# bxh1/VIDO-SLAM

Hardware: AMD Instinct MI355X
Metric: frames/sec end-to-end (flow+depth+track+local-BA) at 640x480; BA iters/sec (higher is better)
Workload: dtype f32

## Files before the change

include/vido_c.h:

```cpp
#ifndef VIDO_C_H
#define VIDO_C_H
#include <stdint.h>
#include <stddef.h>
#ifdef __cplusplus
extern "C" {
#endif

#define VIDO_OK              0
#define VIDO_E_INVALID      -1
#define VIDO_E_NO_DEVICE    -2
#define VIDO_E_HIP          -3
#define VIDO_E_CAPACITY     -4
#define VIDO_E_NOMEM        -5

#define VIDO_MAX_LEVELS 16

typedef struct vido_ctx vido_ctx;

typedef struct vido_keypoint { float x, y, size, angle, response; int32_t octave; } vido_keypoint;

typedef struct vido_config {
    int32_t device;
    int32_t width, height;
    int32_t max_batch;
// ... 152 lines not shown
int vido_conv1x1_set_arith(int arith);
int vido_conv1x1_range_flag(vido_ctx* ctx, int reset);
int vido_conv1x1_bias_act(vido_ctx* ctx, const float* x, const float* w_packed, const float* bias, const float* residual, float* y, int cin, int cout, int hw, float slope);
int vido_deconv2x2_supported(int n, int cin, int cout, int h, int w);
int vido_deconv2x2_bias_act(vido_ctx* ctx, const float* x, const float* w_packed, const float* bias, float* y, int n, int cin, int cout, int h, int w, float slope);
int vido_conv1x1_bias_up2_act(vido_ctx* ctx, const float* x, const float* w_packed, const float* bias, const float* residual_half, float* y, int cin, int cout, int h, int w, float slope);

int vido_conv_kxk_c2(vido_ctx* ctx, const float* x, const float* w, const float* bias, const float* residual, float* y, int cin, int k, int h, int w_);
int vido_conv1x1_skinny(vido_ctx* ctx, const float* x, const float* w_packed, const float* bias, const float* residual, float* y, int cin, int cout, long long hw, float slope);

int vido_conv_direct_supported(int cin, int cout, int h, int w, int kh, int kw, int sh, int sw, int ph, int pw);
long long vido_conv_direct_packed_floats(int cin, int cout, int kh, int kw);
int vido_conv_direct_pack(const float* w, int cin, int cout, int kh, int kw, float* w_packed);
int vido_conv_direct_bias_act(vido_ctx* ctx, const float* x, const float* w_packed, const float* bias, float* y, int n, int cin, int cout, int h, int w,
                              int kh, int kw, int sh, int sw, int ph, int pw, float slope);

int vido_wino3x3_supported(int cin, int cout, int h, int w);
int vido_wino3x3_fills_chip(int n, int cout, int h, int w, int min_wgs);
long long vido_wino3x3_packed_floats(int cin, int cout);
int vido_wino3x3_pack(const float* w, int cin, int cout, float* u_packed);
int vido_wino3x3_bias_act(vido_ctx* ctx, const float* x, const float* u_packed, const float* bias, float* y, int n, int cin, int cout, int h, int w, float slope);
int vido_wino3x3_form(int n, int cin, int cout, int h, int w);
int vido_fc_h_splitk(int rows, int k, int outs);
int vido_fc_h(vido_ctx* ctx, const float* x, const void* w_packed, const float* bias, float* part, float* y, int rows, int k, int outs, float slope);
int vido_conv3x3_h_supported(int n, int cin, int cout, int h, int w);
int vido_conv3x3_h_workgroups(int n, int cout, int h, int w);
int vido_conv3x3_h_bias_act(vido_ctx* ctx, const float* x, const void* w_packed, const float* bias, float* y, int n, int cin, int cout, int h, int w, float slope);
long long vido_wino3x3_packed_floats_form(int cin, int cout, int form);
int vido_wino3x3_pack_form(const float* w, int cin, int cout, int form, float* u_packed);
int vido_wino3x3_bias_act_form(vido_ctx* ctx, const float* x, const float* u_packed, const float* bias, float* y, int n, int cin, int cout, int h, int w, float slope, int form);
int vido_gconv3x3_supported(int H, int W, int cpg_in, int cpg_out);
int64_t vido_gconv3x3_packed_size(int groups, int cpg_in, int cpg_out);
int vido_gconv3x3_bias_act(vido_ctx* ctx, const float* x, const float* in_bias, const float* w_packed, const float* bias, float* y, int groups, int cpg_in, int cpg_out, int H, int W, float slope);
int vido_gconv3x3_s2_supported(int H, int W, int cpg_in, int cpg_out);
int vido_gconv3x3_s2_bias_act(vido_ctx* ctx, const float* x, const float* w_packed, const float* bias, float* y, int groups, int cpg_in, int cpg_out, int H, int W, float slope);
int vido_lfn_reg_front(vido_ctx* ctx, const float* im1, const float* im2, const float* flow, const float* mean, float scale, int B, int C, int H, int W, float* out, int out_channels);
int vido_lfn_reg_tail(vido_ctx* ctx, const float* dist, const float* flow, const float* wx, const float* bx, const float* wy, const float* by, int B, int K, int H, int W, float* out);
int vido_roi_align(vido_ctx* ctx, const float* feat, int B, int C, int H, int W, const float* rois, int n_rois,
                   float spatial_scale, int pooled_h, int pooled_w, int sampling_ratio, float* out, int on_device);
int vido_nms(vido_ctx* ctx, const float* boxes_xyxy, const float* scores, int n, float thresh, int32_t* keep_out,
             int32_t* n_keep, int on_device);
int vido_nms_grouped(vido_ctx* ctx, const float* boxes_xyxy, const float* scores, const int32_t* groups, int n, float thresh,
                     int32_t* keep_out, int32_t* n_keep, int on_device);
int vido_nms_segments(vido_ctx* ctx, const float* boxes_xyxy, const int32_t* groups, const int32_t* seg_off, const int32_t* seg_n, int n_seg, int max_n, int total,
                      float thresh, int32_t* keep_out, int32_t* n_keep);
int vido_roi_align_fpn(vido_ctx* ctx, const float* const feat[4], const int H[4], const int W[4], const float scale[4], int C, const float* boxes, const int32_t* level,
                       int n, int pooled_h, int pooled_w, int sampling_ratio, float* out);
int vido_nchw_to_nhwc(vido_ctx* ctx, const float* src, int B, int C, int H, int W, float* dst);
int vido_roi_align_fpn_nhwc(vido_ctx* ctx, const float* const feat[4], const int H[4], const int W[4], const float scale[4], int C, const float* boxes, const int32_t* level,
                            int n, int pooled_h, int pooled_w, int sampling_ratio, float* out);
int vido_bawin_create(vido_ctx* ctx, int cap_frames, int cap_features);
int vido_bawin_push_frame(vido_ctx* ctx, int frame, int n, const double* meas, const float* xyz, const int32_t* asso);
int vido_bawin_set_labels(vido_ctx* ctx, int n, const int32_t* quads);
int vido_bawin_solve(vido_ctx* ctx, int start, int N, vido_ba_problem* prob, vido_ba_result* res, int32_t* n_obs_out, int32_t* n_pt_out);
int vido_bawin_read_points(vido_ctx* ctx, int frame, int n, float* xyz_out);
int vido_rpn_select(vido_ctx* ctx, int n_levels, const float* const* logits, const float* const* deltas, const int* h, const int* w, const int* stride, const float* cell_anchors,
                    int A, int K, int img_w, int img_h, float* boxes_out, float* scores_out, int32_t* n_out);
int vido_rpn_merge(vido_ctx* ctx, const float* boxes, const float* scores, const int32_t* keep, const int32_t* cnt, int n_levels, int K, int post_nms_top_n, int n_final,
                   float* out_boxes, float* out_scores, int32_t* n_valid);
int vido_det_class_sort(vido_ctx* ctx, const float* prob, const float* deltas, const float* proposals, const float* objectness, int N, int nc, float thresh, const float weights[4],
                        int img_w, int img_h, float* seg_boxes, int32_t* order, int32_t* seg_n);
int vido_det_select(vido_ctx* ctx, const float* prob, const float* seg_boxes, const int32_t* order, const int32_t* keep, const int32_t* cnt, int N, int nc, int detections_per_img, int cap,
                    int32_t* scratch, float* out_boxes, float* out_scores, int64_t* out_labels, int32_t* n_det);
int vido_mask_label_image(vido_ctx* ctx, const float* masks, const float* boxes, const int64_t* labels, int n, int M, int padding, float thresh, int H, int W, uint8_t* out);
int vido_box_decode(vido_ctx* ctx, const float* deltas, const float* boxes, int n, int k, const float weights[4],
                    float* out, int on_device);
// ... 62 lines not shown
```

vido-slam_amd/csrc/conv3x3h.hip:

```cpp
#include "common.hpp"
#include <type_traits>

namespace {
typedef float f32x16 __attribute__((ext_vector_type(16)));
typedef float f32x2 __attribute__((ext_vector_type(2)));
typedef _Float16 f16x8 __attribute__((ext_vector_type(8)));
typedef _Float16 f16x2 __attribute__((ext_vector_type(2)));
typedef unsigned u32x4 __attribute__((ext_vector_type(4)));

#define C3_OOB 0x40000000u
#define C3_WSLOT 24576
#define C3_RBW 3
#define C3_WPIX(BR) (((BR) + 2) * 18)
#define C3_XP(BR) ((16 * C3_WPIX(BR) + 511) / 512)
#define C3_RAW(BR) (C3_XP(BR) * 8 * 256)
#define C3_PLANE(BR) (C3_WPIX(BR) * 32)
#define C3_PBUF(BR) (2 * C3_PLANE(BR))
#define C3_LDS(BR) (C3_RBW * C3_WSLOT + C3_RAW(BR) + 2 * C3_PBUF(BR))

struct C3Args { const float* x; const void* wp; const float* bias; float* y; int N, Cin, Cout, H, W, nby, nbx, mt, total, nchunk; float slope; unsigned xbytes, wbytes; unsigned* range_flag; };

template <int RPW, int CG>
__global__ __launch_bounds__(512) void k_conv3x3_h(C3Args A)
{
    constexpr int BR = 16 / CG, MT = 32 * RPW * CG, WPIX = C3_WPIX(BR), XP = C3_XP(BR), RAWB = C3_RAW(BR), PLANE = C3_PLANE(BR), PBUF = C3_PBUF(BR), CK = (WPIX * 8 + 511) / 512, NMM = 9 * RPW, NRD = 2 * RPW + 2;
    extern __shared__ __attribute__((aligned(16))) char c3_lds[];
    char* L = c3_lds;
    const int tid = threadIdx.x, lane = tid & 63, w = __builtin_amdgcn_readfirstlane(tid >> 6);
    const int per = gridDim.x >> 3, item = (blockIdx.x & 7) * per + (blockIdx.x >> 3);
    if (item >= A.total) return;
    const int nt = item / A.mt, mtile = item - nt * A.mt, m0 = mtile * MT;
    const int bpi = A.nby * A.nbx, n = nt / bpi, brem = nt - n * bpi, by = brem / A.nbx, bx = brem - by * A.nbx, Y0 = by * BR, X0 = bx * 16;
    const int rp = CG == 1 ? w : (w & 3), rb0 = CG == 1 ? 0 : RPW * (w >> 2);
    const int hw = A.H * A.W, nsteps = A.nchunk * 3;

    const __amdgpu_buffer_rsrc_t wr = __builtin_amdgcn_make_buffer_rsrc((void*)A.wp, 0, A.wbytes, 0x00020000);
    const unsigned avo = 16u * (unsigned)lane;
    unsigned abase[3], avq[3];
#pragma unroll
    for (int q = 0; q < 3; q++) { const int i = w + 8 * q, rb = i / 6, rem = i - 6 * rb; abase[q] = 1024u * (unsigned)(((m0 >> 5) + rb) * A.nchunk * 18 + rem); avq[q] = rb < RPW * CG ? avo : 0x80000000u; }
    unsigned xvo[11];
#pragma unroll
    for (int j = 0; j < XP; j++) {
        const int e = 64 * (8 * j + w) + lane, ch = e / WPIX, rem = e - ch * WPIX, row = rem / 18, col = rem - row * 18, gy = Y0 - 1 + row, gx = X0 - 1 + col;
        xvo[j] = (e < 16 * WPIX && gy >= 0 && gy < A.H && gx >= 0 && gx < A.W) ? 4u * (unsigned)(ch * hw + gy * A.W + gx) : C3_OOB;
    }
    const unsigned ximg = 4u * (unsigned)n * (unsigned)A.Cin * (unsigned)hw, xchunk = 64u * (unsigned)hw;
    char* const RAW = L + C3_RBW * C3_WSLOT;
    char* const PL = RAW + RAWB;
    auto issue_w = [&](int s, int slot) {
        char* S = L + slot * C3_WSLOT + w * 1024;
        const unsigned so = 6144u * (unsigned)s;
#pragma unroll
        for (int q = 0; q < 3; q++) __builtin_amdgcn_raw_ptr_buffer_load_lds(wr, (__attribute__((address_space(3))) void*)(S + q * 8192), 16, avq[q], abase[q] + so, 0, 0);
    };
    auto issue_x = [&](int c) {
        const unsigned so = ximg + xchunk * (unsigned)c;
        const __amdgpu_buffer_rsrc_t xc = __builtin_amdgcn_make_buffer_rsrc((void*)((const char*)A.x + so), 0, A.xbytes - so, 0x00020000);
#pragma unroll
        for (int j = 0; j < XP; j++) __builtin_amdgcn_raw_ptr_buffer_load_lds(xc, (__attribute__((address_space(3))) void*)(RAW + (8 * j + w) * 256), 4, xvo[j], 0, 0, 0);
    };
    float xmax = 0.f;
    const f32x2 k2048 = {2048.f, 2048.f};
    auto convert = [&](int buf) {
        const float* R = (const float*)RAW;
        unsigned* P = (unsigned*)(PL + buf * PBUF);
#pragma unroll
        for (int k = 0; k < CK; k++) {
            const int idx = tid + 512 * k;
            if (k < CK - 1 || idx < WPIX * 8) {
                const int q = idx / WPIX, pix = idx - q * WPIX;
                const f32x2 v = {R[(2 * q) * WPIX + pix], R[(2 * q + 1) * WPIX + pix]};
                const f16x2 h = __builtin_convertvector(v, f16x2);
                f32x2 vs, r;
                asm("v_pk_mul_f32 %0, %1, %2" : "=v"(vs) : "v"(v), "v"(k2048));
                asm("v_fma_mix_f32 %0, %1, %2, %3 op_sel_hi:[1,0,0]" : "=v"(r.x) : "v"(h), "s"(-2048.f), "v"(vs.x));
                asm("v_fma_mix_f32 %0, %1, %2, %3 op_sel:[1,0,0] op_sel_hi:[1,0,0]" : "=v"(r.y) : "v"(h), "s"(-2048.f), "v"(vs.y));
                const f16x2 l = __builtin_convertvector(r, f16x2);
                P[pix * 8 + q] = __builtin_bit_cast(unsigned, h); P[PLANE / 4 + pix * 8 + q] = __builtin_bit_cast(unsigned, l);
                xmax = __builtin_fmaxf(__builtin_fmaxf(xmax, __builtin_fabsf(v.x)), __builtin_fabsf(v.y));
            }
        }
    };

    f32x16 acc[RPW], acl[RPW];
#pragma unroll
    for (int rb = 0; rb < RPW; rb++)
#pragma unroll
        for (int r = 0; r < 16; r++) { acc[rb][r] = 0.f; acl[rb][r] = 0.f; }
    typedef const __attribute__((address_space(3))) char* lds_c;
    const unsigned a_lane = 16u * (unsigned)lane;
    const unsigned b_lane = (unsigned)(C3_RBW * C3_WSLOT + RAWB) + 32u * (unsigned)((2 * rp + ((lane & 31) >> 4)) * 18 + (lane & 15)) + 16u * (unsigned)(lane >> 5);

    issue_x(0); issue_w(0, 0); issue_w(min(1, nsteps - 1), 1);
    asm volatile("s_waitcnt vmcnt(6) lgkmcnt(0)\n\ts_barrier" ::: "memory");
    convert(0);
    int slot = 0;
    u32x4 a[2][RPW][2], b[2][2];
    auto step = [&](auto dy_c, auto nbuf_c, int pbuf, auto&& copies) {
        constexpr int dy = decltype(dy_c)::value, NBUF = decltype(nbuf_c)::value;
        lds_c Ab = (lds_c)(L + slot * C3_WSLOT) + a_lane;
        lds_c Bb = (lds_c)L + b_lane + pbuf * PBUF + dy * (18 * 32);
        auto ld = [&](int dx, int set) {
#pragma unroll
            for (int rb = 0; rb < RPW; rb++)
#pragma unroll
                for (int pl = 0; pl < 2; pl++) a[set][rb][pl] = *(const __attribute__((address_space(3))) u32x4*)(Ab + (((rb0 + rb) * 3 + dx) * 2 + pl) * 1024);
#pragma unroll
            for (int pl = 0; pl < 2; pl++) b[set][pl] = *(const __attribute__((address_space(3))) u32x4*)(Bb + dx * 32 + pl * PLANE);
        };
        __builtin_amdgcn_sched_barrier(0);
        ld(0, 0);
        copies();
#pragma unroll
        for (int dx = 0; dx < 3; dx++) {
            if (dx < 2) ld(dx + 1, (dx + 1) & 1);
#pragma unroll
            for (int term = 0; term < 3; term++) {
                constexpr int PA[3] = {0, 1, 0}, PB[3] = {1, 0, 0};
#pragma unroll
                for (int rb = 0; rb < RPW; rb++) {
                    f32x16& d = term == 2 ? acc[rb] : acl[rb];
                    d = __builtin_amdgcn_mfma_f32_32x32x16_f16(__builtin_bit_cast(f16x8, a[dx & 1][rb][PA[term]]), __builtin_bit_cast(f16x8, b[dx & 1][PB[term]]), d, 0, 0, 0);
                }
            }
        }
        __builtin_amdgcn_sched_group_barrier(0x100, NRD, 0);
#pragma unroll
        for (int i = 0; i < NMM; i++) {
            __builtin_amdgcn_sched_group_barrier(0x008, 1, 0);
            if (i < 2 * NRD) __builtin_amdgcn_sched_group_barrier(0x100, 1, 0);
            if (i >= 1 && i < 1 + NBUF) __builtin_amdgcn_sched_group_barrier(0x020, 1, 0);
        }
        __builtin_amdgcn_sched_barrier(0);
    };
    for (int c = 0; c < A.nchunk; c++) {
        const int pbuf = c & 1, cn = min(c + 1, A.nchunk - 1);
        asm volatile("s_waitcnt vmcnt(3) lgkmcnt(0)\n\ts_barrier" ::: "memory");
        step(std::integral_constant<int, 0>{}, std::integral_constant<int, 3 + XP>{}, pbuf, [&] { const int sf = slot == 0 ? C3_RBW - 1 : slot - 1; issue_w(min(3 * c + 2, nsteps - 1), sf); issue_x(cn); });
        slot = slot + 1 == C3_RBW ? 0 : slot + 1;
        asm volatile("s_waitcnt vmcnt(%0) lgkmcnt(0)\n\ts_barrier" :: "n"(3 + XP) : "memory");
        step(std::integral_constant<int, 1>{}, std::integral_constant<int, 3>{}, pbuf, [&] { const int sf = slot == 0 ? C3_RBW - 1 : slot - 1; issue_w(min(3 * c + 3, nsteps - 1), sf); });
        slot = slot + 1 == C3_RBW ? 0 : slot + 1;
        asm volatile("s_waitcnt vmcnt(3) lgkmcnt(0)\n\ts_barrier" ::: "memory");
        step(std::integral_constant<int, 2>{}, std::integral_constant<int, 3>{}, pbuf, [&] { const int sf = slot == 0 ? C3_RBW - 1 : slot - 1; issue_w(min(3 * c + 4, nsteps - 1), sf); });
        convert(pbuf ^ 1);
        slot = slot + 1 == C3_RBW ? 0 : slot + 1;
    }
    asm volatile("s_waitcnt vmcnt(0) lgkmcnt(0)" ::: "memory");
#pragma unroll
    for (int rb = 0; rb < RPW; rb++) acc[rb] += acl[rb] * 0x1p-11f;
    if (!(xmax < 65504.f) && A.range_flag) atomicOr(A.range_flag, 1u);

    const float* wsc = (const float*)((const char*)A.wp + (size_t)A.nchunk * 16 * 18 * A.Cout * 2);
    const int p = lane & 31, Y = Y0 + 2 * rp + (p >> 4), X = X0 + (p & 15);
    const bool inside = Y < A.H && X < A.W;
    float* yb = A.y + (size_t)n * A.Cout * hw + (size_t)Y * A.W + X;
#pragma unroll
    for (int rb = 0; rb < RPW; rb++) {
        float bv[16], sv[16];
#pragma unroll
        for (int r = 0; r < 16; r++) { const int co = m0 + 32 * (rb0 + rb) + 8 * (r >> 2) + 4 * (lane >> 5) + (r & 3); bv[r] = A.bias ? A.bias[co] : 0.f; sv[r] = wsc[co]; }
        if (inside) {
#pragma unroll
            for (int r = 0; r < 16; r++) {
                const int co = m0 + 32 * (rb0 + rb) + 8 * (r >> 2) + 4 * (lane >> 5) + (r & 3);
                const float v = acc[rb][r] * sv[r] + bv[r];
                yb[(size_t)co * hw] = fmaxf(v, v * A.slope);
            }
        }
    }
}
}

extern "C" {

int vido_conv3x3_h_supported(int n, int cin, int cout, int h, int w)
{
    const long long cp = (cin + 15) / 16 * 16;
    return n >= 1 && cin >= 1 && (cout == 32 || cout == 64 || (cout >= 128 && cout % 128 == 0)) && h >= 1 && w >= 1 && 4ll * n * cin * h * w < (1ll << 30) && 4ll * n * cout * h * w < (1ll << 30)
           && 36ll * cp * cout < (1ll << 31);
}

#define C3_MIN16 190
static int c3_block_rows(int n, int cout, int h, int w)
{
    static const int force = [] { const char* e = getenv("VIDO_CONV3X3_H_ROWS"); return e ? atoi(e) : 0; }();
    if (cout == 32) return 16;
    if (force == 16 || force == 8) return force;
    const int mt = cout >= 128 ? cout / 128 : 1;
    return n * ((h + 15) / 16) * ((w + 15) / 16) * mt >= C3_MIN16 ? 16 : 8;
}
int vido_conv3x3_h_workgroups(int n, int cout, int h, int w) { const int br = c3_block_rows(n, cout, h, w); return n * ((h + br - 1) / br) * ((w + 15) / 16) * (cout >= 128 ? cout / 128 : 1); }

int vido_conv3x3_h_bias_act(vido_ctx* ctx, const float* x, const void* w_packed, const float* bias, float* y, int n, int cin, int cout, int h, int w, float slope)
{
    if (!ctx) return VIDO_E_INVALID;
    if (!x || !w_packed || !y || x == y || !vido_conv3x3_h_supported(n, cin, cout, h, w) || slope < 0.f || slope > 1.f || (((uintptr_t)x | (uintptr_t)y) & 3) || ((uintptr_t)w_packed & 15))
        return vido_set_error(ctx, VIDO_E_INVALID, "conv3x3_h: no kernel for %d x %d -> %d channels at %d x %d (or a pointer is misaligned, or slope outside [0, 1])", n, cin, cout, h, w);
    HIP_TRY(ctx, hipSetDevice(ctx->device));
    hipStream_t st = ctx->has_ext_stream ? ctx->ext_stream : ctx->stream;
    const int br = c3_block_rows(n, cout, h, w);
    const int nby = (h + br - 1) / br, nbx = (w + 15) / 16, mt = cout >= 128 ? cout / 128 : 1, total = n * nby * nbx * mt;
    const int nchunk = (cin + 15) / 16;
    C3Args A{x, w_packed, bias, y, n, cin, cout, h, w, nby, nbx, mt, total, nchunk, slope, (unsigned)(4ll * n * cin * h * w), (unsigned)(36ll * 16 * nchunk * cout), ctx->c1_range_flag};
    static bool attr[64] = {};
    if (!attr[ctx->device & 63]) {
#define C3_ATTR(RPW_, CG_) HIP_TRY(ctx, hipFuncSetAttribute((const void*)k_conv3x3_h<RPW_, CG_>, hipFuncAttributeMaxDynamicSharedMemorySize, (int)C3_LDS(16 / CG_)))
        C3_ATTR(4, 1); C3_ATTR(2, 2); C3_ATTR(2, 1); C3_ATTR(1, 2); C3_ATTR(1, 1);
#undef C3_ATTR
        attr[ctx->device & 63] = true;
    }
    const dim3 grid(8 * ((total + 7) / 8));
#define C3_LAUNCH(RPW_, CG_) hipLaunchKernelGGL((k_conv3x3_h<RPW_, CG_>), grid, dim3(512), C3_LDS(16 / CG_), st, A)
    if (cout >= 128) { if (br == 16) C3_LAUNCH(4, 1); else C3_LAUNCH(2, 2); }
    else if (cout == 64) { if (br == 16) C3_LAUNCH(2, 1); else C3_LAUNCH(1, 2); }
    else C3_LAUNCH(1, 1);
#undef C3_LAUNCH
    HIP_TRY(ctx, hipGetLastError());
    return VIDO_OK;
}

}
```

vido-slam_amd/nets/fuse.py:

```python
import os
import torch
import torch.nn as nn
import torch.nn.functional as F


def _fold(conv, bn, eps):
    scale = bn.weight * (bn.running_var + eps).rsqrt()
    w = conv.weight * scale.reshape(-1, 1, 1, 1)
    b = bn.bias - bn.running_mean * scale
    if conv.bias is not None:
        b = b + conv.bias * scale
    return w.detach().contiguous(), b.detach().contiguous()


def _eps(bn):
    return float(getattr(bn, "eps", 0.0))


def fold_batchnorm(net, ops):
    from .maskrcnn import _Bottleneck, _Stem
    from .monodepth2 import _Basic, ResnetEncoder18, DepthDecoder
    n = 0
    for m in net.modules():
        if isinstance(m, _Bottleneck):
            m._w1, m._b1 = _fold(m.conv1, m.bn1, _eps(m.bn1)); m._w2, m._b2 = _fold(m.conv2, m.bn2, _eps(m.bn2)); m._w3, m._b3 = _fold(m.conv3, m.bn3, _eps(m.bn3)); n += 3
            if m.downsample is not None:
                m._wd, m._bd = _fold(m.downsample[0], m.downsample[1], _eps(m.downsample[1])); n += 1
            m._ep = ops.bias_res_act_
            c2 = m.conv2; m._w2p = None; m._ops = ops
            if c2.groups > 1 and tuple(c2.stride) == (1, 1) and tuple(c2.padding) == (1, 1) and tuple(c2.dilation) == (1, 1) and not os.environ.get("VIDO_NO_GCONV"):
                from .ops import pack_gconv3x3
                m._w2p = pack_gconv3x3(m._w2, c2.groups)
            elif (c2.groups > 1 and tuple(c2.stride) == (2, 2) and tuple(c2.padding) == (1, 1) and tuple(c2.dilation) == (1, 1) and ((c2.out_channels // c2.groups) % 32 == 0 or (c2.out_channels // c2.groups) in (8, 16))
                  and not os.environ.get("VIDO_NO_GCONV") and not os.environ.get("VIDO_NO_GCONV_S2")):
                from .ops import pack_gconv3x3
                m._w2p = pack_gconv3x3(m._w2, c2.groups)
            m._w1p = m._w3p = m._wdp = None; m._c1x1_min_tiles = 0
            mode = os.environ.get("VIDO_CONV1X1", "all")
            if not os.environ.get("VIDO_NO_CONV1X1") and hasattr(ops, "conv1x1_bias_act"):
                from .ops import PackedConv1x1
                m._w3p = PackedConv1x1.make(m._w3)
                if mode == "all":
                    if tuple(m.conv1.stride) == (1, 1): m._w1p = PackedConv1x1.make(m._w1)
                    if m.downsample is not None and tuple(m.downsample[0].stride) in ((1, 1), (2, 2)): m._wdp = PackedConv1x1.make(m._wd)
        elif isinstance(m, _Stem):
            m._w1, m._b1 = _fold(m.conv1, m.bn1, _eps(m.bn1)); m._ep = ops.bias_res_act_; n += 1
        elif isinstance(m, _Basic):
            m._w1, m._b1 = _fold(m.conv1, m.bn1, m.bn1.eps); m._w2, m._b2 = _fold(m.conv2, m.bn2, m.bn2.eps); n += 2
            if m.downsample is not None:
                m._wd, m._bd = _fold(m.downsample[0], m.downsample[1], m.downsample[1].eps); n += 1
            m._ep = ops.bias_res_act_
        elif isinstance(m, DepthDecoder):
            m._ops = ops if hasattr(ops, "upcat_reflect") and not os.environ.get("VIDO_NO_DEPTH_FUSED") else None
        elif isinstance(m, ResnetEncoder18):
            e = m.encoder
            w, b = _fold(e.conv1, e.bn1, e.bn1.eps)
            m._w1, m._b1 = w, b; m._ep = ops.bias_res_act_; n += 1
    return n


class Graphed:

    def __init__(self, fn, example_inputs, warmup=2):
        self.fn = fn
        self.static_in = [x.clone() for x in example_inputs]
# ... 19 lines not shown
```

vido-slam_amd/nets/maskrcnn.py:

```python
import math
import os
from collections import OrderedDict
from dataclasses import dataclass
import numpy as np
import torch
import torch.nn as nn
import torch.nn.functional as F


@dataclass
class MaskRCNNConfig:
    blocks: tuple = (3, 4, 23, 3)
    groups: int = 32
    width_per_group: int = 8
    stride_in_1x1: bool = False
    stem_out: int = 64
    res2_out: int = 256
    fpn_out: int = 256
    anchor_sizes: tuple = (32, 64, 128, 256, 512)
    aspect_ratios: tuple = (0.5, 1.0, 2.0)
    anchor_strides: tuple = (4, 8, 16, 32, 64)
    pre_nms_top_n: int = 1000
    post_nms_top_n: int = 1000
    fpn_post_nms_top_n: int = 1000
# ... 7 lines not shown
    score_thresh: float = 0.05
    nms: float = 0.5
    detections_per_img: int = 100
    bbox_reg_weights: tuple = (10.0, 10.0, 5.0, 5.0)
    mask_resolution: int = 14
    mask_layers: tuple = (256, 256, 256, 256)


class FrozenBatchNorm2d(nn.Module):
    def __init__(self, n):
        super().__init__()
        for name, v in (("weight", torch.ones(n)), ("bias", torch.zeros(n)), ("running_mean", torch.zeros(n)), ("running_var", torch.ones(n))):
            self.register_buffer(name, v)

    def forward(self, x):
        scale = self.weight * self.running_var.rsqrt()
        bias = self.bias - self.running_mean * scale
        return x * scale.reshape(1, -1, 1, 1) + bias.reshape(1, -1, 1, 1)


class _Bottleneck(nn.Module):
    def __init__(self, cin, mid, cout, groups, stride_in_1x1, stride):
        super().__init__()
        self.downsample = None
        if cin != cout:
            self.downsample = nn.Sequential(nn.Conv2d(cin, cout, 1, stride, bias=False), FrozenBatchNorm2d(cout))
        s1, s3 = (stride, 1) if stride_in_1x1 else (1, stride)
        self.conv1 = nn.Conv2d(cin, mid, 1, s1, bias=False); self.bn1 = FrozenBatchNorm2d(mid)
        self.conv2 = nn.Conv2d(mid, mid, 3, s3, 1, bias=False, groups=groups); self.bn2 = FrozenBatchNorm2d(mid)
        self.conv3 = nn.Conv2d(mid, cout, 1, bias=False); self.bn3 = FrozenBatchNorm2d(cout)

    _ep = None
    _w2p = None
    _w1p = _w3p = _wdp = None; _c1x1_min_tiles = 0

    def forward(self, x):
        if self._ep is not None and x.is_cuda:
            ep = self._ep; c1, c2 = self.conv1, self.conv2; ops = self._ops
            b1x = x.shape[0] == 1
            hw_in = x.shape[2] * x.shape[3]
            b1_done = False
            from .ops import conv1x1_fills_chip as fills
            if self._w1p is not None and b1x and ops.conv1x1_supported(x.shape[1], self._w1.shape[0], hw_in) and fills(self._w1.shape[0], hw_in):
                y = ops.conv1x1_bias_act(x.contiguous(), self._w1p, self._b1, None, 0.0); b1_done = True
            else:
                y = F.conv2d(x, self._w1, None, c1.stride)
            if (self._w2p is not None and tuple(c2.stride) == (2, 2)):
                if b1_done and y.shape[0] == 1 and self._ops.gconv3x3_s2_supported(y.shape[2], y.shape[3], c2.in_channels // c2.groups, c2.out_channels // c2.groups):
                    y = self._ops.gconv3x3_s2_bias_act(y, self._w2p, self._b2, c2.groups, 0.0)
                else:
                    y = ep(F.conv2d(y if b1_done else ep(y, self._b1, None, 0.0), self._w2, None, c2.stride, c2.padding, c2.dilation, c2.groups), self._b2, None, 0.0)
            elif self._w2p is not None and y.shape[0] == 1 and self._ops.gconv3x3_supported(y.shape[2], y.shape[3], c2.in_channels // c2.groups, c2.out_channels // c2.groups):
                y = self._ops.gconv3x3_bias_act(y, self._w2p, self._b2, c2.groups, 0.0, in_bias=None if b1_done else self._b1)
            else:
                y = ep(F.conv2d(y if b1_done else ep(y, self._b1, None, 0.0), self._w2, None, c2.stride, c2.padding, c2.dilation, c2.groups), self._b2, None, 0.0)
            if self.downsample is None:
                sc = x
            elif self._wdp is not None and b1x and tuple(self.downsample[0].stride) == (1, 1) and ops.conv1x1_supported(x.shape[1], self._wd.shape[0], hw_in) and fills(self._wd.shape[0], hw_in):
                sc = ops.conv1x1_bias_act(x.contiguous(), self._wdp, self._bd, None, 1.0)
            elif (self._wdp is not None and b1x and tuple(self.downsample[0].stride) == (2, 2) and ops.conv1x1_supported(x.shape[1], self._wd.shape[0], ((x.shape[2] + 1) // 2) * ((x.shape[3] + 1) // 2))
                  and fills(self._wd.shape[0], ((x.shape[2] + 1) // 2) * ((x.shape[3] + 1) // 2))):
                sc = ops.conv1x1_bias_act(x[:, :, ::2, ::2].contiguous(), self._wdp, self._bd, None, 1.0)
            else:
                sc = ep(F.conv2d(x, self._wd, None, self.downsample[0].stride), self._bd, None, 1.0)
            if (self._w3p is not None and y.shape[0] == 1 and ops.conv1x1_supported(y.shape[1], self._w3.shape[0], y.shape[2] * y.shape[3])
                    and (fills(self._w3.shape[0], y.shape[2] * y.shape[3]) or self._c1x1_min_tiles < 0)):
                return ops.conv1x1_bias_act(y.contiguous(), self._w3p, self._b3, sc, 0.0)
            return ep(F.conv2d(y, self._w3), self._b3, sc.contiguous(), 0.0)
        y = F.relu(self.bn1(self.conv1(x)))
        y = F.relu(self.bn2(self.conv2(y)))
        y = self.bn3(self.conv3(y))
        return F.relu(y + (x if self.downsample is None else self.downsample(x)))


class _Stem(nn.Module):
    def __init__(self, cout):
        super().__init__()
        self.conv1 = nn.Conv2d(3, cout, 7, 2, 3, bias=False); self.bn1 = FrozenBatchNorm2d(cout)

    _ep = None

    def forward(self, x):
        if self._ep is not None and x.is_cuda:
            return F.max_pool2d(self._ep(F.conv2d(x, self._w1, None, 2, 3), self._b1, None, 0.0), 3, 2, 1)
# ... 595 lines not shown
```

vido-slam_amd/nets/ops.py:

```python
import ctypes as C
import os
import torch

_WINO_MIN_WGS = int(os.environ.get("VIDO_WINO_MIN_WGS", "0"))
_CONV3X3_H_MIN_WGS = 0 if os.environ.get("VIDO_CONV3X3_H") == "0" else int(os.environ.get("VIDO_CONV3X3_H_MIN_WGS", "128"))
_CONVDIRECT_SET = os.environ.get("VIDO_CONVDIRECT_SET", "novalu")


def correlation_torch_reference(first, second, stride):
    a, b = first[:, :, ::stride, ::stride], second[:, :, ::stride, ::stride]
    pad = torch.nn.functional.pad(b, (3, 3, 3, 3))
    H, W = a.shape[2], a.shape[3]
    return torch.stack([(a * pad[:, :, p:p + H, o:o + W]).mean(1) for p in range(7) for o in range(7)], 1)


class HipOps:

    def __init__(self, ctx):
        self.ctx = ctx

    def _adopt_stream(self):
        st = torch.cuda.current_stream().cuda_stream
        self.ctx._check(self.ctx.lib.vido_set_stream(self.ctx.h, C.c_void_p(st), 1))

# ... 106 lines not shown
        self._adopt_stream()
        self.ctx._check(self.ctx.lib.vido_area_feed(self.ctx.h, C.c_void_p(bgr.data_ptr()), bgr.shape[0], bgr.shape[1], C.c_void_p(out.data_ptr()), int(feed[0]), int(feed[1]), C.c_float(div)))
        return out

    def backwarp(self, x, flow):
        assert x.is_cuda and x.dtype == torch.float32 and flow.dtype == torch.float32 and x.shape[0] == flow.shape[0] and x.shape[2:] == flow.shape[2:] and flow.shape[1] == 2
        x = x.contiguous(); flow = flow.contiguous()
        out = torch.empty_like(x)
        self._adopt_stream()
        self.ctx._check(self.ctx.lib.vido_backwarp(self.ctx.h, C.c_void_p(x.data_ptr()), C.c_void_p(flow.data_ptr()), x.shape[0], x.shape[1], x.shape[2], x.shape[3], C.c_void_p(out.data_ptr())))
        return out

    def deconv4s2_depthwise(self, x, weight, input_slope=1.0):
        x = x.contiguous(); B, Cc, H, W = x.shape
        assert weight.shape == (Cc, 1, 4, 4) and weight.is_contiguous()
        out = torch.empty((B, Cc, 2 * H, 2 * W), device=x.device, dtype=torch.float32)
        self._adopt_stream()
        self.ctx._check(self.ctx.lib.vido_deconv4s2_depthwise(self.ctx.h, C.c_void_p(x.data_ptr()), C.c_void_p(weight.data_ptr()), B, Cc, H, W, C.c_float(input_slope), C.c_void_p(out.data_ptr())))
        return out

    def gconv3x3_supported(self, H, W, cpg_in, cpg_out):
        return bool(self.ctx.lib.vido_gconv3x3_supported(int(H), int(W), int(cpg_in), int(cpg_out)))

    def gconv3x3_bias_act(self, x, w_packed, bias, groups, slope=0.0, in_bias=None):
        assert x.is_cuda and x.is_contiguous() and x.dtype == torch.float32 and x.shape[0] == 1
        _, Cin, H, W = x.shape
        cpg_in = Cin // groups; cpg_out = bias.numel() // groups
        out = torch.empty((1, bias.numel(), H, W), device=x.device, dtype=torch.float32)
        self.gconv_flops = getattr(self, "gconv_flops", 0.0) + 2.0 * bias.numel() * cpg_in * 9 * H * W
        self._adopt_stream()
        self.ctx._check(self.ctx.lib.vido_gconv3x3_bias_act(self.ctx.h, C.c_void_p(x.data_ptr()), C.c_void_p(in_bias.data_ptr()) if in_bias is not None else None,
                                                            C.c_void_p(w_packed.data_ptr()), C.c_void_p(bias.data_ptr()), C.c_void_p(out.data_ptr()),
                                                            int(groups), cpg_in, cpg_out, H, W, C.c_float(slope)))
        return out

    def gconv3x3_s2_supported(self, H, W, cpg_in, cpg_out):
        return bool(self.ctx.lib.vido_gconv3x3_s2_supported(int(H), int(W), int(cpg_in), int(cpg_out)))

    def gconv3x3_s2_bias_act(self, x, w_packed, bias, groups, slope=0.0):
        assert x.is_cuda and x.is_contiguous() and x.dtype == torch.float32 and x.shape[0] == 1
        _, Cin, H, W = x.shape
        cpg_in = Cin // groups; cpg_out = bias.numel() // groups
        out = torch.empty((1, bias.numel(), (H + 1) // 2, W // 2), device=x.device, dtype=torch.float32)
        self.gconv_flops = getattr(self, "gconv_flops", 0.0) + 2.0 * bias.numel() * cpg_in * 9 * out.shape[2] * out.shape[3]
        self._adopt_stream()
        self.ctx._check(self.ctx.lib.vido_gconv3x3_s2_bias_act(self.ctx.h, C.c_void_p(x.data_ptr()), C.c_void_p(w_packed.data_ptr()), C.c_void_p(bias.data_ptr()), C.c_void_p(out.data_ptr()),
                                                               int(groups), cpg_in, cpg_out, H, W, C.c_float(slope)))
        return out

    def conv1x1_supported(self, cin, cout, hw):
        return bool(self.ctx.lib.vido_conv1x1_supported(int(cin), int(cout), int(hw)))

    def conv1x1_set_arith(self, arith):
        return int(self.ctx.lib.vido_conv1x1_set_arith(int(arith)))

    def conv1x1_range_flag(self, reset=True):
        return int(self.ctx.lib.vido_conv1x1_range_flag(self.ctx.h, int(bool(reset))))

    def conv1x1_layout(self, cin, cout, hw):
        return int(self.ctx.lib.vido_conv1x1_layout(int(cin), int(cout), int(hw)))

    def conv1x1_bias_act(self, x, w_packed, bias=None, residual=None, slope=1.0, residual_up2=None):
        assert x.is_cuda and x.is_contiguous() and x.dtype == torch.float32 and x.shape[0] == 1
        _, cin, H, W = x.shape
        if isinstance(w_packed, PackedConv1x1):
            w_packed = w_packed.get(self.conv1x1_layout(cin, w_packed.cout, H * W), x.device)
# ... 364 lines not shown
    m = w.abs().amax(1)
    _, ex = torch.frexp(torch.where(m > 0, m, torch.ones_like(m)))
    e = torch.where(m > 0, 15 - ex, torch.zeros_like(ex)).clamp(-100, 100).to(torch.int32)
    pow2 = lambda k: ((k + 127) << 23).view(torch.float32)
    ws = w * pow2(e)[:, None]
    h = ws.to(torch.float16)
    l = ((ws - h.float()) * 2048.0).to(torch.float16)
    return h, l, pow2(-e)


def pack_conv1x1(w, layout=0):
    cout, cin = int(w.shape[0]), int(w.shape[1])
    if w.dim() == 4 and tuple(w.shape[2:]) != (1, 1):
        return None
    if cout % 128 or cin % 32 or (layout == 1 and cin % 64):
        return None
    if layout == 3:
        h, l, inv = split_f16x2(w.detach().reshape(cout, cin))
        w6 = torch.stack([h, l], 0).view(torch.int16).reshape(2, cout // 32, 32, cin // 16, 2, 8)
        planes = w6.permute(1, 3, 0, 4, 2, 5).contiguous().reshape(-1)
        return torch.cat([planes, inv.contiguous().view(torch.int16).reshape(-1)])
    if layout == 2:
        p0, p1, p2 = split_bf16x3(w.detach().reshape(cout, cin).float())
        w6 = torch.stack([p0, p1, p2], 0).view(torch.int16).reshape(3, cout // 32, 32, cin // 16, 2, 8)
        return w6.permute(1, 3, 0, 4, 2, 5).contiguous().reshape(cout // 32, cin // 16, 3, 64, 8)
    if layout == 1:
        w5 = w.detach().reshape(cout // 16, 16, cin // 16, 4, 4)
        return w5.permute(0, 2, 4, 1, 3).contiguous().reshape(cout // 16, cin // 16, 64, 4)
    w5 = w.detach().reshape(cout // 32, 32, cin // 8, 4, 2)
    return w5.permute(0, 2, 4, 1, 3).contiguous().reshape(cout // 32, cin // 8, 64, 4)


def pack_conv3x3_h(w):
    cout, cin0 = int(w.shape[0]), int(w.shape[1])
    if tuple(w.shape[2:]) != (3, 3) or not (cout in (32, 64) or (cout >= 128 and cout % 128 == 0)):
        return None
    cin = (cin0 + 15) // 16 * 16
    if cin != cin0:
        w = torch.cat([w.detach(), torch.zeros(cout, cin - cin0, 3, 3, dtype=w.dtype, device=w.device)], 1)
    h, l, inv = split_f16x2(w.detach().reshape(cout, cin * 9))
    planes = torch.stack([h, l], 0).view(torch.int16).reshape(2, cout // 32, 32, cin // 16, 2, 8, 3, 3)
    planes = planes.permute(1, 3, 6, 7, 0, 4, 2, 5).contiguous().reshape(-1)
    return torch.cat([planes, inv.contiguous().view(torch.int16).reshape(-1)])


def pack_deconv2x2(w):
    cin, cout = int(w.shape[0]), int(w.shape[1])
    wm = w.detach().permute(2, 3, 1, 0).reshape(4 * cout, cin, 1, 1)
    return pack_conv1x1(wm, 3)


class PackedConv1x1:

    def __init__(self, w):
        self.w = w.detach(); self.cout = int(w.shape[0]); self.cin = int(w.shape[1]); self._p = {}

    @staticmethod
    def make(w):
        return PackedConv1x1(w) if pack_conv1x1(w, 0) is not None else None

    def get(self, layout, device):
        key = (int(layout), str(device))
        if key not in self._p:
            p = pack_conv1x1(self.w, layout)
            assert p is not None, "conv1x1: layout %d does not take %d -> %d channels" % (layout, self.cin, self.cout)
            self._p[key] = p.to(device)
        return self._p[key]


# ... 54 lines not shown
```

Baseline: 131.5.

## Route grouped 3x3 convs through split-f16 MFMA conv3x3_h kernel with per-group weights

Reuses the split-f16 matrix-core 3x3 conv kernel for grouped convolutions by treating each group as a batch image with its own weight block (gblk offset), adding C API and Python wrappers, and enabling it by default in ResNeXt blocks. It also adds a smaller-LDS variant for the 32-channel form, with sink slots for unused loads, so two workgroups fit per CU. The aim is to replace the older gconv kernel with a tensor-core path, at the cost of extra packed weights and the split-f16 precision path.

```diff
diff --git a/include/vido_c.h b/include/vido_c.h
--- a/include/vido_c.h
+++ b/include/vido_c.h
@@ -208,6 +208,8 @@
 int vido_gconv3x3_supported(int H, int W, int cpg_in, int cpg_out);
 int64_t vido_gconv3x3_packed_size(int groups, int cpg_in, int cpg_out);
 int vido_gconv3x3_bias_act(vido_ctx* ctx, const float* x, const float* in_bias, const float* w_packed, const float* bias, float* y, int groups, int cpg_in, int cpg_out, int H, int W, float slope);
+int vido_gconv3x3_h_supported(int groups, int cpg_in, int cpg_out, int H, int W);
+int vido_gconv3x3_h_bias_act(vido_ctx* ctx, const float* x, const void* w_packed, const float* bias, float* y, int groups, int cpg_in, int cpg_out, int H, int W, float slope);
 int vido_gconv3x3_s2_supported(int H, int W, int cpg_in, int cpg_out);
 int vido_gconv3x3_s2_bias_act(vido_ctx* ctx, const float* x, const float* w_packed, const float* bias, float* y, int groups, int cpg_in, int cpg_out, int H, int W, float slope);
 int vido_lfn_reg_front(vido_ctx* ctx, const float* im1, const float* im2, const float* flow, const float* mean, float scale, int B, int C, int H, int W, float* out, int out_channels);
diff --git a/vido-slam_amd/csrc/conv3x3h.hip b/vido-slam_amd/csrc/conv3x3h.hip
--- a/vido-slam_amd/csrc/conv3x3h.hip
+++ b/vido-slam_amd/csrc/conv3x3h.hip
@@ -16,14 +16,21 @@
 #define C3_RAW(BR) (C3_XP(BR) * 8 * 256)
 #define C3_PLANE(BR) (C3_WPIX(BR) * 32)
 #define C3_PBUF(BR) (2 * C3_PLANE(BR))
-#define C3_LDS(BR) (C3_RBW * C3_WSLOT + C3_RAW(BR) + 2 * C3_PBUF(BR))
-
-struct C3Args { const float* x; const void* wp; const float* bias; float* y; int N, Cin, Cout, H, W, nby, nbx, mt, total, nchunk; float slope; unsigned xbytes, wbytes; unsigned* range_flag; };
+#define C3_SMALL(RPW, CG) ((RPW) * (CG) == 1)
+#define C3_WS(RPW, CG) (C3_SMALL(RPW, CG) ? 6144 : C3_WSLOT)
+#define C3_NW(RPW, CG) (C3_SMALL(RPW, CG) ? 1 : 3)
+#define C3_RAWF(RPW, CG) (C3_SMALL(RPW, CG) ? 64 * C3_WPIX(16 / (CG)) : C3_RAW(16 / (CG)))
+#define C3_LDS(RPW, CG) (C3_RBW * C3_WS(RPW, CG) + C3_RAWF(RPW, CG) + 2 * C3_PBUF(16 / (CG)) + (C3_SMALL(RPW, CG) ? 1024 : 0))
+static_assert(C3_LDS(1, 1) <= 80 * 1024, "two workgroups of the 32-channel form per CU");
+
+struct C3Args { const float* x; const void* wp; const float* bias; float* y; int N, Cin, Cout, H, W, nby, nbx, mt, total, nchunk; float slope; unsigned xbytes, wbytes; unsigned* range_flag; int gblk; };
 
 template <int RPW, int CG>
 __global__ __launch_bounds__(512) void k_conv3x3_h(C3Args A)
 {
-    constexpr int BR = 16 / CG, MT = 32 * RPW * CG, WPIX = C3_WPIX(BR), XP = C3_XP(BR), RAWB = C3_RAW(BR), PLANE = C3_PLANE(BR), PBUF = C3_PBUF(BR), CK = (WPIX * 8 + 511) / 512, NMM = 9 * RPW, NRD = 2 * RPW + 2;
+    constexpr int BR = 16 / CG, MT = 32 * RPW * CG, WPIX = C3_WPIX(BR), XP = C3_XP(BR), RAWB = C3_RAWF(RPW, CG), PLANE = C3_PLANE(BR), PBUF = C3_PBUF(BR), CK = (WPIX * 8 + 511) / 512, NMM = 9 * RPW, NRD = 2 * RPW + 2;
+    constexpr bool SMALL = C3_SMALL(RPW, CG);
+    constexpr int WS = C3_WS(RPW, CG), NW = C3_NW(RPW, CG);
     extern __shared__ __attribute__((aligned(16))) char c3_lds[];
     char* L = c3_lds;
     const int tid = threadIdx.x, lane = tid & 63, w = __builtin_amdgcn_readfirstlane(tid >> 6);
@@ -38,7 +45,7 @@
     const unsigned avo = 16u * (unsigned)lane;
     unsigned abase[3], avq[3];
 #pragma unroll
-    for (int q = 0; q < 3; q++) { const int i = w + 8 * q, rb = i / 6, rem = i - 6 * rb; abase[q] = 1024u * (unsigned)(((m0 >> 5) + rb) * A.nchunk * 18 + rem); avq[q] = rb < RPW * CG ? avo : 0x80000000u; }
+    for (int q = 0; q < 3; q++) { const int i = w + 8 * q, rb = i / 6, rem = i - 6 * rb; abase[q] = 1024u * (unsigned)(((m0 >> 5) + n * A.gblk + rb) * A.nchunk * 18 + rem); avq[q] = rb < RPW * CG ? avo : 0x80000000u; }
     unsigned xvo[11];
 #pragma unroll
     for (int j = 0; j < XP; j++) {
@@ -46,19 +53,22 @@
         xvo[j] = (e < 16 * WPIX && gy >= 0 && gy < A.H && gx >= 0 && gx < A.W) ? 4u * (unsigned)(ch * hw + gy * A.W + gx) : C3_OOB;
     }
     const unsigned ximg = 4u * (unsigned)n * (unsigned)A.Cin * (unsigned)hw, xchunk = 64u * (unsigned)hw;
-    char* const RAW = L + C3_RBW * C3_WSLOT;
+    char* const RAW = L + C3_RBW * WS;
     char* const PL = RAW + RAWB;
+    char* const SINK = PL + 2 * PBUF;
     auto issue_w = [&](int s, int slot) {
-        char* S = L + slot * C3_WSLOT + w * 1024;
+        char* S = L + slot * WS + w * 1024;
         const unsigned so = 6144u * (unsigned)s;
 #pragma unroll
-        for (int q = 0; q < 3; q++) __builtin_amdgcn_raw_ptr_buffer_load_lds(wr, (__attribute__((address_space(3))) void*)(S + q * 8192), 16, avq[q], abase[q] + so, 0, 0);
+        for (int q = 0; q < NW; q++)
+            __builtin_amdgcn_raw_ptr_buffer_load_lds(wr, (__attribute__((address_space(3))) void*)(SMALL && w >= 6 ? SINK : S + q * 8192), 16, avq[q], abase[q] + so, 0, 0);
     };
     auto issue_x = [&](int c) {
         const unsigned so = ximg + xchunk * (unsigned)c;
         const __amdgpu_buffer_rsrc_t xc = __builtin_amdgcn_make_buffer_rsrc((void*)((const char*)A.x + so), 0, A.xbytes - so, 0x00020000);
 #pragma unroll
-        for (int j = 0; j < XP; j++) __builtin_amdgcn_raw_ptr_buffer_load_lds(xc, (__attribute__((address_space(3))) void*)(RAW + (8 * j + w) * 256), 4, xvo[j], 0, 0, 0);
+        for (int j = 0; j < XP; j++)
+            __builtin_amdgcn_raw_ptr_buffer_load_lds(xc, (__attribute__((address_space(3))) void*)(SMALL && (8 * j + w) * 256 >= RAWB ? SINK : RAW + (8 * j + w) * 256), 4, xvo[j], 0, 0, 0);
     };
     float xmax = 0.f;
     const f32x2 k2048 = {2048.f, 2048.f};
@@ -90,16 +100,16 @@
         for (int r = 0; r < 16; r++) { acc[rb][r] = 0.f; acl[rb][r] = 0.f; }
     typedef const __attribute__((address_space(3))) char* lds_c;
     const unsigned a_lane = 16u * (unsigned)lane;
-    const unsigned b_lane = (unsigned)(C3_RBW * C3_WSLOT + RAWB) + 32u * (unsigned)((2 * rp + ((lane & 31) >> 4)) * 18 + (lane & 15)) + 16u * (unsigned)(lane >> 5);
+    const unsigned b_lane = (unsigned)(C3_RBW * WS + RAWB) + 32u * (unsigned)((2 * rp + ((lane & 31) >> 4)) * 18 + (lane & 15)) + 16u * (unsigned)(lane >> 5);
 
     issue_x(0); issue_w(0, 0); issue_w(min(1, nsteps - 1), 1);
-    asm volatile("s_waitcnt vmcnt(6) lgkmcnt(0)\n\ts_barrier" ::: "memory");
+    asm volatile("s_waitcnt vmcnt(%0) lgkmcnt(0)\n\ts_barrier" :: "n"(2 * NW) : "memory");
     convert(0);
     int slot = 0;
     u32x4 a[2][RPW][2], b[2][2];
     auto step = [&](auto dy_c, auto nbuf_c, int pbuf, auto&& copies) {
         constexpr int dy = decltype(dy_c)::value, NBUF = decltype(nbuf_c)::value;
-        lds_c Ab = (lds_c)(L + slot * C3_WSLOT) + a_lane;
+        lds_c Ab = (lds_c)(L + slot * WS) + a_lane;
         lds_c Bb = (lds_c)L + b_lane + pbuf * PBUF + dy * (18 * 32);
         auto ld = [&](int dx, int set) {
 #pragma unroll
@@ -136,14 +146,14 @@
     };
     for (int c = 0; c < A.nchunk; c++) {
         const int pbuf = c & 1, cn = min(c + 1, A.nchunk - 1);
-        asm volatile("s_waitcnt vmcnt(3) lgkmcnt(0)\n\ts_barrier" ::: "memory");
-        step(std::integral_constant<int, 0>{}, std::integral_constant<int, 3 + XP>{}, pbuf, [&] { const int sf = slot == 0 ? C3_RBW - 1 : slot - 1; issue_w(min(3 * c + 2, nsteps - 1), sf); issue_x(cn); });
+        asm volatile("s_waitcnt vmcnt(%0) lgkmcnt(0)\n\ts_barrier" :: "n"(NW) : "memory");
+        step(std::integral_constant<int, 0>{}, std::integral_constant<int, NW + XP>{}, pbuf, [&] { const int sf = slot == 0 ? C3_RBW - 1 : slot - 1; issue_w(min(3 * c + 2, nsteps - 1), sf); issue_x(cn); });
         slot = slot + 1 == C3_RBW ? 0 : slot + 1;
-        asm volatile("s_waitcnt vmcnt(%0) lgkmcnt(0)\n\ts_barrier" :: "n"(3 + XP) : "memory");
-        step(std::integral_constant<int, 1>{}, std::integral_constant<int, 3>{}, pbuf, [&] { const int sf = slot == 0 ? C3_RBW - 1 : slot - 1; issue_w(min(3 * c + 3, nsteps - 1), sf); });
+        asm volatile("s_waitcnt vmcnt(%0) lgkmcnt(0)\n\ts_barrier" :: "n"(NW + XP) : "memory");
+        step(std::integral_constant<int, 1>{}, std::integral_constant<int, NW>{}, pbuf, [&] { const int sf = slot == 0 ? C3_RBW - 1 : slot - 1; issue_w(min(3 * c + 3, nsteps - 1), sf); });
         slot = slot + 1 == C3_RBW ? 0 : slot + 1;
-        asm volatile("s_waitcnt vmcnt(3) lgkmcnt(0)\n\ts_barrier" ::: "memory");
-        step(std::integral_constant<int, 2>{}, std::integral_constant<int, 3>{}, pbuf, [&] { const int sf = slot == 0 ? C3_RBW - 1 : slot - 1; issue_w(min(3 * c + 4, nsteps - 1), sf); });
+        asm volatile("s_waitcnt vmcnt(%0) lgkmcnt(0)\n\ts_barrier" :: "n"(NW) : "memory");
+        step(std::integral_constant<int, 2>{}, std::integral_constant<int, NW>{}, pbuf, [&] { const int sf = slot == 0 ? C3_RBW - 1 : slot - 1; issue_w(min(3 * c + 4, nsteps - 1), sf); });
         convert(pbuf ^ 1);
         slot = slot + 1 == C3_RBW ? 0 : slot + 1;
     }
@@ -152,7 +162,8 @@
     for (int rb = 0; rb < RPW; rb++) acc[rb] += acl[rb] * 0x1p-11f;
     if (!(xmax < 65504.f) && A.range_flag) atomicOr(A.range_flag, 1u);
 
-    const float* wsc = (const float*)((const char*)A.wp + (size_t)A.nchunk * 16 * 18 * A.Cout * 2);
+    const float* wsc = (const float*)((const char*)A.wp + A.wbytes);
+    const int cw0 = m0 + 32 * n * A.gblk;
     const int p = lane & 31, Y = Y0 + 2 * rp + (p >> 4), X = X0 + (p & 15);
     const bool inside = Y < A.H && X < A.W;
     float* yb = A.y + (size_t)n * A.Cout * hw + (size_t)Y * A.W + X;
@@ -160,7 +171,7 @@
     for (int rb = 0; rb < RPW; rb++) {
         float bv[16], sv[16];
 #pragma unroll
-        for (int r = 0; r < 16; r++) { const int co = m0 + 32 * (rb0 + rb) + 8 * (r >> 2) + 4 * (lane >> 5) + (r & 3); bv[r] = A.bias ? A.bias[co] : 0.f; sv[r] = wsc[co]; }
+        for (int r = 0; r < 16; r++) { const int co = cw0 + 32 * (rb0 + rb) + 8 * (r >> 2) + 4 * (lane >> 5) + (r & 3); bv[r] = A.bias ? A.bias[co] : 0.f; sv[r] = wsc[co]; }
         if (inside) {
 #pragma unroll
             for (int r = 0; r < 16; r++) {
@@ -193,26 +204,24 @@
 }
 int vido_conv3x3_h_workgroups(int n, int cout, int h, int w) { const int br = c3_block_rows(n, cout, h, w); return n * ((h + br - 1) / br) * ((w + 15) / 16) * (cout >= 128 ? cout / 128 : 1); }
 
-int vido_conv3x3_h_bias_act(vido_ctx* ctx, const float* x, const void* w_packed, const float* bias, float* y, int n, int cin, int cout, int h, int w, float slope)
-{
-    if (!ctx) return VIDO_E_INVALID;
-    if (!x || !w_packed || !y || x == y || !vido_conv3x3_h_supported(n, cin, cout, h, w) || slope < 0.f || slope > 1.f || (((uintptr_t)x | (uintptr_t)y) & 3) || ((uintptr_t)w_packed & 15))
-        return vido_set_error(ctx, VIDO_E_INVALID, "conv3x3_h: no kernel for %d x %d -> %d channels at %d x %d (or a pointer is misaligned, or slope outside [0, 1])", n, cin, cout, h, w);
+static int c3_run(vido_ctx* ctx, const float* x, const void* w_packed, const float* bias, float* y, int n, int cin, int cout, int h, int w, float slope, int gblk)
+{
     HIP_TRY(ctx, hipSetDevice(ctx->device));
     hipStream_t st = ctx->has_ext_stream ? ctx->ext_stream : ctx->stream;
     const int br = c3_block_rows(n, cout, h, w);
     const int nby = (h + br - 1) / br, nbx = (w + 15) / 16, mt = cout >= 128 ? cout / 128 : 1, total = n * nby * nbx * mt;
     const int nchunk = (cin + 15) / 16;
-    C3Args A{x, w_packed, bias, y, n, cin, cout, h, w, nby, nbx, mt, total, nchunk, slope, (unsigned)(4ll * n * cin * h * w), (unsigned)(36ll * 16 * nchunk * cout), ctx->c1_range_flag};
+    const long long wcout = gblk ? (long long)n * cout : cout;
+    C3Args A{x, w_packed, bias, y, n, cin, cout, h, w, nby, nbx, mt, total, nchunk, slope, (unsigned)(4ll * n * cin * h * w), (unsigned)(36ll * 16 * nchunk * wcout), ctx->c1_range_flag, gblk};
     static bool attr[64] = {};
     if (!attr[ctx->device & 63]) {
-#define C3_ATTR(RPW_, CG_) HIP_TRY(ctx, hipFuncSetAttribute((const void*)k_conv3x3_h<RPW_, CG_>, hipFuncAttributeMaxDynamicSharedMemorySize, (int)C3_LDS(16 / CG_)))
+#define C3_ATTR(RPW_, CG_) HIP_TRY(ctx, hipFuncSetAttribute((const void*)k_conv3x3_h<RPW_, CG_>, hipFuncAttributeMaxDynamicSharedMemorySize, (int)C3_LDS(RPW_, CG_)))
         C3_ATTR(4, 1); C3_ATTR(2, 2); C3_ATTR(2, 1); C3_ATTR(1, 2); C3_ATTR(1, 1);
 #undef C3_ATTR
         attr[ctx->device & 63] = true;
     }
     const dim3 grid(8 * ((total + 7) / 8));
-#define C3_LAUNCH(RPW_, CG_) hipLaunchKernelGGL((k_conv3x3_h<RPW_, CG_>), grid, dim3(512), C3_LDS(16 / CG_), st, A)
+#define C3_LAUNCH(RPW_, CG_) hipLaunchKernelGGL((k_conv3x3_h<RPW_, CG_>), grid, dim3(512), C3_LDS(RPW_, CG_), st, A)
     if (cout >= 128) { if (br == 16) C3_LAUNCH(4, 1); else C3_LAUNCH(2, 2); }
     else if (cout == 64) { if (br == 16) C3_LAUNCH(2, 1); else C3_LAUNCH(1, 2); }
     else C3_LAUNCH(1, 1);
@@ -221,4 +230,27 @@
     return VIDO_OK;
 }
 
-}
+int vido_conv3x3_h_bias_act(vido_ctx* ctx, const float* x, const void* w_packed, const float* bias, float* y, int n, int cin, int cout, int h, int w, float slope)
+{
+    if (!ctx) return VIDO_E_INVALID;
+    if (!x || !w_packed || !y || x == y || !vido_conv3x3_h_supported(n, cin, cout, h, w) || slope < 0.f || slope > 1.f || (((uintptr_t)x | (uintptr_t)y) & 3) || ((uintptr_t)w_packed & 15))
+        return vido_set_error(ctx, VIDO_E_INVALID, "conv3x3_h: no kernel for %d x %d -> %d channels at %d x %d (or a pointer is misaligned, or slope outside [0, 1])", n, cin, cout, h, w);
+    return c3_run(ctx, x, w_packed, bias, y, n, cin, cout, h, w, slope, 0);
+}
+
+int vido_gconv3x3_h_supported(int groups, int cpg_in, int cpg_out, int h, int w)
+{
+    const long long cp = (cpg_in + 15) / 16 * 16;
+    return groups >= 1 && (cpg_out == 32 || cpg_out == 64) && vido_conv3x3_h_supported(groups, cpg_in, cpg_out, h, w) && 36ll * cp * cpg_out * groups < (1ll << 31);
+}
+
+int vido_gconv3x3_h_bias_act(vido_ctx* ctx, const float* x, const void* w_packed, const float* bias, float* y, int groups, int cpg_in, int cpg_out, int h, int w, float slope)
+{
+    if (!ctx) return VIDO_E_INVALID;
+    if (!x || !w_packed || !y || x == y || !vido_gconv3x3_h_supported(groups, cpg_in, cpg_out, h, w) || slope < 0.f || slope > 1.f || (((uintptr_t)x | (uintptr_t)y) & 3)
+        || ((uintptr_t)w_packed & 15))
+        return vido_set_error(ctx, VIDO_E_INVALID, "gconv3x3_h: no kernel for %d groups of %d -> %d channels at %d x %d (or a pointer is misaligned, or slope outside [0, 1])", groups, cpg_in, cpg_out, h, w);
+    return c3_run(ctx, x, w_packed, bias, y, groups, cpg_in, cpg_out, h, w, slope, cpg_out / 32);
+}
+
+}
diff --git a/vido-slam_amd/nets/fuse.py b/vido-slam_amd/nets/fuse.py
--- a/vido-slam_amd/nets/fuse.py
+++ b/vido-slam_amd/nets/fuse.py
@@ -27,10 +27,12 @@
             if m.downsample is not None:
                 m._wd, m._bd = _fold(m.downsample[0], m.downsample[1], _eps(m.downsample[1])); n += 1
             m._ep = ops.bias_res_act_
-            c2 = m.conv2; m._w2p = None; m._ops = ops
+            c2 = m.conv2; m._w2p = m._w2h = None; m._ops = ops
             if c2.groups > 1 and tuple(c2.stride) == (1, 1) and tuple(c2.padding) == (1, 1) and tuple(c2.dilation) == (1, 1) and not os.environ.get("VIDO_NO_GCONV"):
-                from .ops import pack_gconv3x3
+                from .ops import pack_gconv3x3, pack_gconv3x3_h
                 m._w2p = pack_gconv3x3(m._w2, c2.groups)
+                if os.environ.get("VIDO_GCONV_H", "1") != "0":
+                    m._w2h = pack_gconv3x3_h(m._w2, c2.groups)
             elif (c2.groups > 1 and tuple(c2.stride) == (2, 2) and tuple(c2.padding) == (1, 1) and tuple(c2.dilation) == (1, 1) and ((c2.out_channels // c2.groups) % 32 == 0 or (c2.out_channels // c2.groups) in (8, 16))
                   and not os.environ.get("VIDO_NO_GCONV") and not os.environ.get("VIDO_NO_GCONV_S2")):
                 from .ops import pack_gconv3x3
diff --git a/vido-slam_amd/nets/maskrcnn.py b/vido-slam_amd/nets/maskrcnn.py
--- a/vido-slam_amd/nets/maskrcnn.py
+++ b/vido-slam_amd/nets/maskrcnn.py
@@ -63,6 +63,7 @@
 
     _ep = None
     _w2p = None
+    _w2h = None
     _w1p = _w3p = _wdp = None; _c1x1_min_tiles = 0
 
     def forward(self, x):
@@ -81,6 +82,9 @@
                     y = self._ops.gconv3x3_s2_bias_act(y, self._w2p, self._b2, c2.groups, 0.0)
                 else:
                     y = ep(F.conv2d(y if b1_done else ep(y, self._b1, None, 0.0), self._w2, None, c2.stride, c2.padding, c2.dilation, c2.groups), self._b2, None, 0.0)
+            elif (self._w2h is not None and b1_done and y.shape[0] == 1
+                  and ops.gconv3x3_h_supported(c2.groups, c2.in_channels // c2.groups, c2.out_channels // c2.groups, y.shape[2], y.shape[3])):
+                y = ops.gconv3x3_h_bias_act(y.contiguous(), self._w2h, self._b2, c2.groups, 0.0)
             elif self._w2p is not None and y.shape[0] == 1 and self._ops.gconv3x3_supported(y.shape[2], y.shape[3], c2.in_channels // c2.groups, c2.out_channels // c2.groups):
                 y = self._ops.gconv3x3_bias_act(y, self._w2p, self._b2, c2.groups, 0.0, in_bias=None if b1_done else self._b1)
             else:
diff --git a/vido-slam_amd/nets/ops.py b/vido-slam_amd/nets/ops.py
--- a/vido-slam_amd/nets/ops.py
+++ b/vido-slam_amd/nets/ops.py
@@ -162,6 +162,21 @@
         self.ctx._check(self.ctx.lib.vido_gconv3x3_bias_act(self.ctx.h, C.c_void_p(x.data_ptr()), C.c_void_p(in_bias.data_ptr()) if in_bias is not None else None,
                                                             C.c_void_p(w_packed.data_ptr()), C.c_void_p(bias.data_ptr()), C.c_void_p(out.data_ptr()),
                                                             int(groups), cpg_in, cpg_out, H, W, C.c_float(slope)))
+        return out
+
+    def gconv3x3_h_supported(self, groups, cpg_in, cpg_out, H, W):
+        return bool(self.ctx.lib.vido_gconv3x3_h_supported(int(groups), int(cpg_in), int(cpg_out), int(H), int(W)))
+
+    def gconv3x3_h_bias_act(self, x, w_packed, bias, groups, slope=0.0):
+        assert x.is_cuda and x.is_contiguous() and x.dtype == torch.float32 and x.shape[0] == 1
+        _, Cin, H, W = x.shape
+        cout = bias.numel(); cpg_in = Cin // groups; cpg_out = cout // groups
+        assert w_packed.dtype == torch.int16 and w_packed.numel() == 2 * cout * ((cpg_in + 15) // 16 * 16 * 9 + 1), "gconv3x3_h: weight not packed by pack_gconv3x3_h for this layer"
+        out = torch.empty((1, cout, H, W), device=x.device, dtype=torch.float32)
+        self.gconv_flops = getattr(self, "gconv_flops", 0.0) + 2.0 * cout * cpg_in * 9 * H * W
+        self._adopt_stream()
+        self.ctx._check(self.ctx.lib.vido_gconv3x3_h_bias_act(self.ctx.h, C.c_void_p(x.data_ptr()), C.c_void_p(w_packed.data_ptr()), C.c_void_p(bias.data_ptr()),
+                                                              C.c_void_p(out.data_ptr()), int(groups), cpg_in, cpg_out, H, W, C.c_float(slope)))
         return out
 
     def gconv3x3_s2_supported(self, H, W, cpg_in, cpg_out):
@@ -592,9 +607,20 @@
 
 
 def pack_conv3x3_h(w):
-    cout, cin0 = int(w.shape[0]), int(w.shape[1])
+    cout = int(w.shape[0])
     if tuple(w.shape[2:]) != (3, 3) or not (cout in (32, 64) or (cout >= 128 and cout % 128 == 0)):
         return None
+    return _pack_3x3_split_f16(w)
+
+
+def pack_gconv3x3_h(w, groups):
+    if tuple(w.shape[2:]) != (3, 3) or int(w.shape[0]) % groups or int(w.shape[0]) // groups not in (32, 64):
+        return None
+    return _pack_3x3_split_f16(w)
+
+
+def _pack_3x3_split_f16(w):
+    cout, cin0 = int(w.shape[0]), int(w.shape[1])
     cin = (cin0 + 15) // 16 * 16
     if cin != cin0:
         w = torch.cat([w.detach(), torch.zeros(cout, cin - cin0, 3, 3, dtype=w.dtype, device=w.device)], 1)
```

Measured after the change: 132.9 (median of 6 runs). 1.01x the previous value.
